# zpelgrims/pota

Measured on AMD Instinct MI355X. Metric: bidir redistribution Msamples/s at 4K, double-gauss 50mm, higher is better.
Workload: dtype f64

## Files before the change

include/lentil_hip.h:

```cpp
#ifndef LENTIL_HIP_H
#define LENTIL_HIP_H

#include <stddef.h>
#include <stdint.h>

#ifdef __cplusplus
extern "C" {
#endif

#define LENTIL_ABI_VERSION 1

#define LENTIL_OK 0
#define LENTIL_ERR_INVALID (-1)
#define LENTIL_ERR_HIP (-2)
#define LENTIL_ERR_UNSUPPORTED (-3)
#define LENTIL_ERR_NOMEM (-4)

#define LENTIL_THINLENS 0
#define LENTIL_POLYNOMIAL_OPTICS 1
#define LENTIL_UNIT_MM 0
#define LENTIL_UNIT_CM 1
#define LENTIL_UNIT_DM 2
#define LENTIL_UNIT_M 3
#define LENTIL_FILTER_GAUSSIAN 0
// ... 208 lines not shown

int lentil_hip_accum_buffer(lentil_hip_ctx *ctx, void **device_ptr, uint64_t *n_floats);
int lentil_hip_stream(lentil_hip_ctx *ctx, void **hip_stream);

int lentil_hip_comm_unique_id(uint8_t id[128]);
int lentil_hip_comm_init(lentil_hip_ctx *ctx, const uint8_t id[128], int rank, int world);
int lentil_hip_comm_destroy(lentil_hip_ctx *ctx);
int lentil_hip_allreduce(lentil_hip_ctx *ctx);
int lentil_hip_exchange_bands(lentil_hip_ctx *ctx, const int32_t *bounds, int32_t visit_rows, int32_t sparse,
                              int32_t *band_lo, int32_t *band_hi);
int lentil_hip_exchange_stats(lentil_hip_ctx *ctx, uint64_t *bytes_sent, uint64_t *bytes_received);
int lentil_hip_exchange_counts(lentil_hip_ctx *ctx, uint64_t *fixed_form, uint64_t *pairs_overflowed);
int lentil_hip_degenerate_stats(lentil_hip_ctx *ctx, uint32_t *degenerate, uint64_t *flagged_pixels, uint64_t *nodes_sent,
                                uint64_t *nodes_received, uint64_t *passes_rerun);
int lentil_hip_streams_concurrent(lentil_hip_ctx *ctx, int *concurrent);
int lentil_hip_box_probe(lentil_hip_ctx *ctx, double probe[6]);

typedef struct lentil_crypto_visits {
  uint64_t n;
  uint32_t n_crypto;
  uint32_t entries;
  const float *hash[LENTIL_MAX_CRYPTO];
  const float *weight[LENTIL_MAX_CRYPTO];
} lentil_crypto_visits;
int lentil_hip_alloc_crypto(lentil_hip_ctx *ctx, uint32_t n_crypto, uint32_t slots_per_pixel);
int lentil_hip_upload_crypto(lentil_hip_ctx *ctx, const lentil_crypto_visits *c);
int lentil_hip_bind_crypto(lentil_hip_ctx *ctx, const lentil_crypto_visits *c);
int lentil_hip_visits_begin_crypto(lentil_hip_ctx *ctx, uint32_t entries);
int lentil_hip_visits_append_crypto(lentil_hip_ctx *ctx, const lentil_visits *part, const lentil_crypto_visits *caches,
                                    uint64_t *ticket);
int lentil_hip_download_crypto(lentil_hip_ctx *ctx, uint32_t crypto, uint32_t rank, float *host_rgba, uint8_t *host_has_rank);
int lentil_hip_download_crypto_table(lentil_hip_ctx *ctx, uint32_t crypto, uint32_t *slots_per_pixel, uint32_t *host_id_bits,
                                     float *host_weight, float *host_total);

int lentil_hip_get_counters(lentil_hip_ctx *ctx, lentil_counters *out);
int lentil_hip_last_timing(lentil_hip_ctx *ctx, float ms[3]);
int lentil_hip_last_launches(lentil_hip_ctx *ctx, uint32_t n[2]);
int lentil_hip_batch_model_stats(lentil_hip_ctx *ctx, uint64_t stats[4]);
int lentil_hip_process_stats(uint64_t stats[4]);
int lentil_hip_process_stall_notes(char *buf, uint64_t capacity);
typedef struct lentil_probe_segment {
  float origin[3];
  float target[3];
} lentil_probe_segment;
typedef void (*lentil_probe_fn)(void *user, uint64_t n, const lentil_probe_segment *segments, uint8_t *occluded);
int lentil_hip_set_occlusion_probe(lentil_hip_ctx *ctx, lentil_probe_fn fn, void *user, const float *camera_to_world);
int lentil_hip_probe_stats(lentil_hip_ctx *ctx, uint64_t stats[3]);

int lentil_hip_set_async(lentil_hip_ctx *ctx, int on);
int lentil_hip_pass_totals(lentil_hip_ctx *ctx, lentil_pass_totals *out, int reset);
int lentil_hip_debug_batch_estimate(lentil_hip_ctx *ctx, uint64_t n, const float *cs_xyz, uint32_t samples, float *out);
int lentil_hip_set_draw_log(lentil_hip_ctx *ctx, uint64_t capacity);
int lentil_hip_download_draw_log(lentil_hip_ctx *ctx, lentil_draw_record *out, uint64_t capacity,
                                 uint64_t *n_records);

#define LENTIL_RAYS_DEVICE_POINTERS 1u
#define LENTIL_RAYS_NO_DIFFERENTIALS 2u
typedef struct lentil_camera_ray_batch {
  uint64_t n;
  uint64_t first_ray;
  const float *in;
  float *out;
  int32_t *tries;
  double lambda;
  float exposure;
  uint32_t rng_seed;
  uint32_t flags;
} lentil_camera_ray_batch;
int lentil_hip_camera_rays(lentil_hip_ctx *ctx, const lentil_camera_ray_batch *batch);
int lentil_hip_camera_rays_path(lentil_hip_ctx *ctx, int *path);

int lentil_hip_test_y0_intersection(lentil_hip_ctx *ctx, uint64_t n, const double *sensor_shift, double lambda,
                                    double *distance, double *sensor, double *out);
int lentil_hip_test_lt_sample_aperture(lentil_hip_ctx *ctx, uint64_t n, const double *scene,
                                       const double *ap, double lambda, double *sensor,
                                       double *out, double *transmittance);
int lentil_hip_test_trace_bw_po(lentil_hip_ctx *ctx, uint64_t n, const double *target,
                                const int32_t *px, const int32_t *py, const int32_t *attempt,
                                double *sensor_xy, int32_t *ok);
int lentil_hip_test_aperture_sample(lentil_hip_ctx *ctx, uint64_t n, const uint32_t *a,
                                    const uint32_t *b, double *xy);
int lentil_hip_test_xor128_jump(const uint32_t in[4], uint64_t k, uint32_t out[4]);
int lentil_hip_debug_scan_bands(const lentil_params *params, float out[8]);
enum {
  LENTIL_SCAN_DMA2 = 1,
  LENTIL_SCAN_DMA = 2,
  LENTIL_SCAN_DMA_MULTI = 3,
  LENTIL_SCAN_UNIFORM = 4,
  LENTIL_SCAN_UNIFORM_MULTI = 5,
  LENTIL_SCAN_RUNS = 6,
  LENTIL_SCAN_RAGGED = 7
};
int lentil_hip_debug_last_scan(lentil_hip_ctx *ctx, uint32_t out[4]);

#ifdef __cplusplus
}
#endif
#endif
```

pota_amd/capi.py:

```python
import ctypes as C
import os

import numpy as np

from . import _abi

_PKG = os.path.dirname(os.path.abspath(__file__))
LIB_PATH = os.environ.get("LENTIL_HIP_LIB") or os.path.join(_PKG, "liblentil_hip.so")

EXPORTS = [
    "lentil_hip_abi_version", "lentil_hip_create", "lentil_hip_destroy", "lentil_hip_last_error", "lentil_hip_last_redo_note",
    "lentil_hip_set_params", "lentil_hip_set_lens", "lentil_hip_set_bokeh", "lentil_hip_alloc_frame", "lentil_hip_set_camera_motion", "lentil_hip_set_camera_shutter",
    "lentil_hip_upload_visits", "lentil_hip_bind_visits", "lentil_hip_clear_frame",
    "lentil_hip_redistribute", "lentil_hip_resolve", "lentil_hip_sync", "lentil_hip_download_aov",
    "lentil_hip_download_accum", "lentil_hip_download_records", "lentil_hip_accum_buffer", "lentil_hip_stream",
    "lentil_hip_set_closest_exchange", "lentil_hip_zkey_buffer", "lentil_hip_closest_gather",
    "lentil_hip_touched_rows", "lentil_hip_merge_rows", "lentil_hip_resolve_rows",
    "lentil_hip_pack_rows", "lentil_hip_merge_packed_rows", "lentil_hip_compact_rows", "lentil_hip_merge_sparse",
    "lentil_hip_get_counters", "lentil_hip_last_timing", "lentil_hip_last_launches", "lentil_hip_set_draw_log",
    "lentil_hip_batch_model_stats", "lentil_hip_process_stats", "lentil_hip_process_stall_notes", "lentil_hip_set_async", "lentil_hip_pass_totals", "lentil_hip_set_occlusion_probe", "lentil_hip_probe_stats", "lentil_hip_debug_batch_estimate", "lentil_hip_box_probe",
    "lentil_hip_lens_jit_status", "lentil_hip_lens_jit_wait", "lentil_hip_debug_lens_jit_source", "lentil_hip_debug_lens_jit_compile",
    "lentil_hip_download_draw_log", "lentil_hip_test_lt_sample_aperture",
    "lentil_hip_test_trace_bw_po", "lentil_hip_test_aperture_sample", "lentil_hip_debug_scan_bands", "lentil_hip_debug_last_scan",
    "lentil_hip_lens_is_compiled", "lentil_hip_set_lens_mode",
    "lentil_hip_focus_search", "lentil_hip_test_y0_intersection", "lentil_hip_camera_rays", "lentil_hip_camera_rays_path",
    "lentil_hip_set_xor128_state", "lentil_hip_get_xor128_state", "lentil_hip_tl_chroma_stats", "lentil_hip_test_xor128_jump",
    "lentil_hip_host_alloc", "lentil_hip_host_free", "lentil_hip_visits_begin", "lentil_hip_visits_append",
    "lentil_hip_visits_wait", "lentil_hip_visits_end",
    "lentil_hip_comm_unique_id", "lentil_hip_comm_init", "lentil_hip_comm_destroy", "lentil_hip_allreduce",
    "lentil_hip_exchange_bands", "lentil_hip_exchange_stats", "lentil_hip_exchange_counts", "lentil_hip_degenerate_stats", "lentil_hip_streams_concurrent",
    "lentil_hip_alloc_crypto", "lentil_hip_upload_crypto", "lentil_hip_bind_crypto", "lentil_hip_download_crypto",
    "lentil_hip_download_crypto_table", "lentil_hip_visits_begin_crypto", "lentil_hip_visits_append_crypto",
]

SCAN_DMA2, SCAN_DMA, SCAN_DMA_MULTI, SCAN_UNIFORM, SCAN_UNIFORM_MULTI, SCAN_RUNS, SCAN_RAGGED = range(1, 8)
SCAN_NAMES = {SCAN_DMA2: "dma2", SCAN_DMA: "dma", SCAN_DMA_MULTI: "dma_multi", SCAN_UNIFORM: "uniform",
              SCAN_UNIFORM_MULTI: "uniform_multi", SCAN_RUNS: "runs", SCAN_RAGGED: "ragged"}

_lib = None


def process_stats():
    lib = load_library()
    n = (C.c_uint64 * 4)()
    rc = lib.lentil_hip_process_stats(n)
    if rc:
        raise RuntimeError("lentil_hip_process_stats: %d" % rc)
    return tuple(int(x) for x in n)


def process_stall_notes():
    lib = load_library()
    buf = C.create_string_buffer(1 << 14)
    lib.lentil_hip_process_stall_notes(buf, 1 << 14)
    return buf.value.decode(errors="replace")


def _tea8(v0, v1):
    v0 = np.asarray(v0, np.uint32).copy()
    v1 = np.broadcast_to(np.asarray(v1, np.uint32), v0.shape).copy()
    s0 = np.uint32(0)
    with np.errstate(over="ignore"):
        for _ in range(8):
            s0 = np.uint32((int(s0) + 0x9E3779B9) & 0xFFFFFFFF)
            v0 += ((v1 << np.uint32(4)) + np.uint32(0xA341316C)) ^ (v1 + s0) ^ ((v1 >> np.uint32(5)) + np.uint32(0xC8013EA4))
            v1 += ((v0 << np.uint32(4)) + np.uint32(0xAD90777D)) ^ (v0 + s0) ^ ((v0 >> np.uint32(5)) + np.uint32(0x7E95761E))
    return v0


def ray_rng_state(ray_id, seed):
    rid = np.asarray(ray_id, np.uint32)
    w = [_tea8(rid, np.uint32(int(seed) & 0xFFFFFFFF))]
    for _ in range(3):
        w.append(_tea8(rid, w[-1]))
    st = np.stack(w, -1)
    st[~st.any(-1)] = np.array([123456789, 362436069, 521288629, 88675123], np.uint32)
    return st


class LentilError(RuntimeError):
    def __init__(self, code, msg):
        super().__init__("lentil_hip error %d: %s" % (code, msg))
        self.code = code


def load_library():
    global _lib
    if _lib is not None:
        return _lib
    if os.environ.get("LENTIL_NO_TORCH") != "1":
        try:
            import torch
        except ImportError:
            pass
    if not os.path.exists(LIB_PATH):
        raise FileNotFoundError(
            "%s is missing: build it with `python -c 'import __graft_entry__ as g; g.build()'`" % LIB_PATH)
    lib = C.CDLL(LIB_PATH)
    vp, u32, u64, i = C.c_void_p, C.c_uint32, C.c_uint64, C.c_int
    sig = {
        "lentil_hip_abi_version": (i, []),
        "lentil_hip_create": (i, [i, C.POINTER(vp)]),
        "lentil_hip_destroy": (i, [vp]),
        "lentil_hip_last_error": (C.c_char_p, [vp]),
        "lentil_hip_last_redo_note": (C.c_char_p, [vp]),
        "lentil_hip_set_params": (i, [vp, C.POINTER(_abi.Params)]),
# ... 584 lines not shown
```

pota_amd/csrc/lentil_hip.hip:

```cpp
#include <hip/hip_runtime.h>
#include <hip/hip_ext.h>

#include <algorithm>
#include <atomic>
#include <chrono>
#include <cmath>
#include <cstdio>
#include <cstdlib>
#include <cstring>
#include <deque>
#include <mutex>
#include <new>
#include <string>
#include <vector>

#include "lentil_kernels.h"
#include "lentil_closest_replay.h"
#include "lentil_tl_chroma_mgpu.h"
#include "lentil_lens_jit.h"
#include "lentil_camera_rays.h"
#include "generated/embedded_sources.inc"

#define LENTIL_API extern "C" __attribute__((visibility("default")))

// ... 1738 lines not shown
  int rc;
  if (ctx->F.dir && (rc = fold_direct(ctx, 0, ctx->F.np, true))) return rc;
  if (ctx->dir_dirty && !(region && *region == ctx->dir_region)) {
    const lentil_hip_ctx::DirRegion &r = ctx->dir_region;
    const uint64_t rows = r.ppr ? (r.npix + r.ppr - 1) / r.ppr : 0;
    uint64_t row_lo = (uint64_t)(r.y0 < 0 ? 0 : r.y0);
    uint64_t row_hi = rows ? row_lo + (rows - 1) * (r.row_stride ? r.row_stride : 1) + 1 : row_lo;
    if (row_hi > ctx->P.yres) row_hi = ctx->P.yres;
    if (row_hi > row_lo)
      HIP_TRY(ctx, hipMemsetAsync(ctx->d_dir + row_lo * ctx->P.xres * ctx->F.stride, 0,
                                  (row_hi - row_lo) * ctx->P.xres * ctx->F.stride * sizeof(float), ctx->stream));
    ctx->dir_dirty = false;
  }
  if (region) {
    if (!ctx->d_dir) {
      const uint64_t nfl = ctx->F.np * ctx->F.stride;
      HIP_TRY(ctx, hipMalloc(&ctx->d_dir, nfl * sizeof(float)));
      HIP_TRY(ctx, hipMemsetAsync(ctx->d_dir, 0, nfl * sizeof(float), ctx->stream));
    }
    ctx->F.dir = ctx->d_dir;
    ctx->dir_dirty = true;
    ctx->dir_region = *region;
    if (ctx->cleared_since_pass) {
      if (!ctx->d_touched) {
        const uint64_t n = touched_bytes(ctx->F.np);
        HIP_TRY(ctx, hipMalloc(&ctx->d_touched, n));
        HIP_TRY(ctx, hipMemsetAsync(ctx->d_touched, 0, n, ctx->stream));
      }
      ctx->F.touched = ctx->d_touched;
      ctx->F.touched_px = ctx->d_touched + touched_px_offset(ctx->F.np);
    }
  } else {
    untrust_touched(ctx);
  }
  ctx->cleared_since_pass = false;
  return LENTIL_OK;
}

static ScanBands scan_bands(const lentil_params &P) {
  ScanBands B;
  for (int i = 0; i < 2; ++i) { B.in_lo[i] = 1.0f; B.in_hi[i] = -1.0f; B.out_lo[i] = 1.0f; B.out_hi[i] = -1.0f; }
  B.out_lo[0] = -INFINITY; B.out_hi[0] = INFINITY;
  float fd = (float)P.focus_distance, A = (float)P.aperture_radius;
  if (P.cameraType == LENTIL_POLYNOMIAL_OPTICS) fd = (float)((double)fd / 10.0);
  else A = (float)((double)A * 10.0);
  const float f = P.focal_length;
  const float ifd = (-f * -fd) / (-f + -fd);
  const double a = std::fabs((double)A), c0 = 1.0 + (double)ifd / (double)f, c1 = (double)ifd;
  if (!(a > 0.0) || !std::isfinite(a) || !std::isfinite(c0) || !std::isfinite(c1) || c1 == 0.0 || !(f > 0.0f)) return B;
  const double eps = 1e-3 + 1e-5 * a;
  if (!(eps < 0.25)) return B;
  auto up = [](double v) { float r = (float)v; if ((double)r < v) r = std::nextafter(r, INFINITY); return r; };
  auto down = [](double v) { float r = (float)v; if ((double)r > v) r = std::nextafter(r, -INFINITY); return r; };
  auto pieces = [&](double t, bool inner, float lo[2], float hi[2]) {
    double ua = (c0 - t / a) / c1, ub = (c0 + t / a) / c1;
    if (ua > ub) std::swap(ua, ub);
    lo[0] = lo[1] = 1.0f; hi[0] = hi[1] = -1.0f;
    const double big = inner ? 1e30 : (double)INFINITY;
    if (ua > 0.0 || ub < 0.0) {
      const double zl = 1.0 / ub, zh = 1.0 / ua;
      lo[0] = inner ? up(std::max(zl, -big)) : down(zl);
      hi[0] = inner ? down(std::min(zh, big)) : up(zh);
    } else {
      if (ua < 0.0) { lo[0] = inner ? (float)-big : -INFINITY; hi[0] = inner ? down(1.0 / ua) : up(1.0 / ua); }
      if (ub > 0.0) { lo[1] = inner ? up(1.0 / ub) : down(1.0 / ub); hi[1] = inner ? (float)big : INFINITY; }
      if (!inner && (ua == 0.0 || ub == 0.0)) { lo[0] = -INFINITY; hi[0] = INFINITY; }
    }
  };
  ScanBands R = B;
  pieces(0.4 * (1.0 - eps), true, R.in_lo, R.in_hi);
  pieces(0.4 * (1.0 + eps), false, R.out_lo, R.out_hi);
  for (int i = 0; i < 2; ++i)
    if (std::isnan(R.in_lo[i]) || std::isnan(R.in_hi[i]) || std::isnan(R.out_lo[i]) || std::isnan(R.out_hi[i])) return B;
  return R;
}

LENTIL_API int lentil_hip_debug_scan_bands(const lentil_params *P, float out[8]) {
  if (!P || !out) return LENTIL_ERR_INVALID;
  const ScanBands B = scan_bands(*P);
  for (int i = 0; i < 2; ++i) { out[i] = B.in_lo[i]; out[2 + i] = B.in_hi[i]; out[4 + i] = B.out_lo[i]; out[6 + i] = B.out_hi[i]; }
  return LENTIL_OK;
}

struct ScanPlan {
  ScanArgs sa{};
  size_t lds = 0;
  uint64_t n_tiles = 0;
  bool multi = false;
  bool dma = false;
  bool dma2 = false;
  bool dma_multi = false;
  uint32_t M = 0;
};

static uint32_t dma_multi_ring(const lentil_hip_ctx *) {
  static const int forced = getenv("LENTIL_DMA_MULTI_RING") ? atoi(getenv("LENTIL_DMA_MULTI_RING")) : 0;
  return forced == 3 ? 3u : 2u;
}
static uint32_t dma_multi_blocks_per_cu(const lentil_hip_ctx *ctx) {
  static const int forced = getenv("LENTIL_DMA_MULTI_BLOCKS") ? atoi(getenv("LENTIL_DMA_MULTI_BLOCKS")) : 0;
  if (forced >= 1 && forced <= 4) return (uint32_t)forced;
  const size_t one = (size_t)4 * dma_multi_wave_f4(ctx->V.n_extra, dma_multi_ring(ctx)) * 16 + 4 * kWaveQueueLds * sizeof(uint2);
  return 2u * one + 2u * 10u * 1024u <= 160u * 1024u ? 2u : 1u;
}
static size_t dma_multi_lds(const lentil_hip_ctx *ctx) {
  return (size_t)4 * dma_multi_wave_f4(ctx->V.n_extra, dma_multi_ring(ctx)) * 16 + 4 * kWaveQueueLds * sizeof(uint2);
}

static bool dma_multi_applies(const lentil_hip_ctx *ctx) {
  static const bool allowed = !(getenv("LENTIL_SCAN_DMA_MULTI") && getenv("LENTIL_SCAN_DMA_MULTI")[0] == '0');
  const uint32_t M = ctx->V.visits_per_pixel;
  return allowed && ctx->scan_dma && M > 0 && M <= 64 && ctx->V.n_extra > 0 && !ctx->V.inv_density && !ctx->F.zkey && !ctx->F.zkey_dbg &&
         ctx->F.closest_mask == 0 && ctx->V.cam.n < 2 && ctx->V.n % M == 0 && dma_multi_lds(ctx) <= 160u * 1024u;
}

static size_t solve_block_lds(lentil_hip_ctx *ctx) {
  const bool straight = ctx->use_generated && (lentil_hip_lens_is_compiled(ctx) || jit_function(ctx, false, true) != nullptr);
  return straight ? 29184u : 53760u;
}

static int plan_scan(lentil_hip_ctx *ctx, ScanPlan &pl) {
  ScanArgs &sa = pl.sa;
  sa.P = ctx->P;
  sa.lens_length = ctx->have_lens ? ctx->hlens.length : 0.0;
  sa.V = ctx->V;
  sa.F = ctx->F;
  const uint32_t M = ctx->V.visits_per_pixel;
  pl.M = M;
  if (M) {
    uint32_t ppt = 64;
    uint64_t lds_budget = (ctx->V.n_extra ? 24ull : 48ull) * 1024ull;
    if (const char *e = getenv("LENTIL_SCAN_LDS_KB")) lds_budget = strtoull(e, nullptr, 10) * 1024ull;
    while (ppt > 1 && (uint64_t)ppt * M * 20ull * 4ull > lds_budget) ppt >>= 1;
    if ((uint64_t)ppt * M * 20ull * 4ull > 150ull * 1024ull)
      return fail(ctx, LENTIL_ERR_UNSUPPORTED, "visits_per_pixel too large for the LDS staging area");
    sa.ppt = ppt;
    sa.tv_pad = ppt * M;
    pl.lds = (size_t)sa.tv_pad * 20 * 4 + 4 * kWaveQueueLds * sizeof(uint2);
    pl.multi = ctx->V.n_extra > 0 && M <= 64 && !getenv("LENTIL_SCAN_SINGLE_COLUMN");
    if (pl.multi) {
      ppt = 64 / M;
      sa.ppt = ppt;
      sa.tv_pad = ppt * M;
      const size_t wave_f4 = (size_t)ctx->F.n_aovs * kMultiPlane + 16 + (size_t)ppt * (ctx->F.stride / 4);
      pl.lds = 4 * wave_f4 * 16 + 4 * kWaveQueueLds * sizeof(uint2);
    }
    uint32_t dma_ring = kDmaRing;
    if (const char *e = getenv("LENTIL_DMA_RING")) { const int r = atoi(e); if (r >= 2 && r <= 8) dma_ring = (uint32_t)r; }
    const size_t dma_lds = (size_t)4 * dma_wave_f4(M, dma_ring) * 16 + 4 * kWaveQueueLds * sizeof(uint2);
    pl.dma = ctx->scan_dma && ctx->V.n_extra == 0 && !ctx->V.inv_density && !ctx->F.zkey && !ctx->F.zkey_dbg && ctx->V.cam.n < 2 &&
             ctx->V.n % M == 0 && dma_lds <= 80u * 1024u;
    if (pl.dma) {
      ppt = 64;
      sa.ring = dma_ring;
      sa.ppt = ppt;
      sa.tv_pad = ppt * M;
      pl.lds = dma_lds;
      pl.multi = false;
      static const bool dma2_allowed = !(getenv("LENTIL_SCAN_DMA2") && getenv("LENTIL_SCAN_DMA2")[0] == '0');
      const size_t dma2_lds = (size_t)4 * dma2_wave_f4(M) * 16 + 4 * kWaveQueueLds * sizeof(uint2);
      const size_t solve_lds = (size_t)ctx->stream_blocks * solve_block_lds(ctx);
      const uint64_t ppr = ctx->V.pixels_per_row;
      pl.dma2 = dma2_allowed && M >= 2 && ppr >= 2 && ppr < (1ull << 31) && ctx->V.n / M < (1ull << 31) &&
                dma2_lds + (ctx->stream_mode ? solve_lds : 0) <= 160u * 1024u;
      if (pl.dma2) {
        pl.lds = dma2_lds;
// ... 2436 lines not shown
```

pota_amd/csrc/lentil_kernels.h:

```cpp
#pragma once
#include "lentil_device.h"
#include "lentil_batch_model.h"
#include "generated/lens_registry.h"

using namespace lentil;

struct DevCounters {
  unsigned long long work_count;
  unsigned long long sum_samples;
  unsigned long long redistributed;
  unsigned long long attempted;
  unsigned long long accepted;
  unsigned long long overflow;
  unsigned long long log_count;
  unsigned long long newton_iters;
  unsigned long long tries;
  unsigned long long lane_rounds;
  unsigned long long slow_solves;
  unsigned long long fallback;
  unsigned long long rounds_used;
  unsigned int n_tasks[2];
  unsigned int task_head[2];
  unsigned int n_active[2];
  unsigned int active_head[2];
// ... 680 lines not shown
  nskip[lane] = 0u;
  auto issue_ring = [&](uint64_t v0, uint32_t g) {
    const uint64_t v = v0 + (uint64_t)g * 64u + lane;
    const uint64_t vl = v < V.n ? v : v_last;
    float4 *slot = ring + (size_t)(g % R) * 192u;
    lds_dma16(V.pos_z + vl, slot);
    lds_dma16(V.volume_ignore + vl, slot + 64);
    lds_dma16(V.transmission + vl, slot + 128);
  };

  while (true) {
    uint32_t t4 = 0;
    if (lane == 0) t4 = atomicAdd(&a.ctr->tile_next, 4u);
    t4 = __builtin_amdgcn_readfirstlane(t4);
    if (a.tile_begin + (uint64_t)t4 >= n_tiles) break;
    const uint64_t tile4 = a.tile_begin + (uint64_t)scan_order(a, t4, 4u);
    const uint64_t tile4_end = tile4 + 4u < n_tiles ? tile4 + 4u : n_tiles;
    for (uint64_t tile = tile4; tile < tile4_end; ++tile) {
      const uint64_t pix0 = tile * 64u;
      const uint64_t v0 = pix0 * M;
      for (uint32_t g = 0; g < M; ++g) {
        const uint64_t v = v0 + (uint64_t)g * 64u + lane;
        lds_dma16(V.rgba + (v < V.n ? v : v_last), srgba + (size_t)g * 64u);
      }
      for (uint32_t g = 0; g < R && g < M; ++g) issue_ring(v0, g);
      for (uint32_t g = 0; g < M; ++g) {
        const uint32_t behind = (M - 1u - g) < (R - 1u) ? (M - 1u - g) : (R - 1u);
        wait_vmcnt(3u * behind);
        float4 pz, vi, tr;
        lds_read_slot(ring + (size_t)(g % R) * 192u + lane, pz, vi, tr);
        const uint32_t e = g * 64u + lane;
        const uint64_t v = v0 + e;
        const bool valid = v < V.n;
        bool flagged = false;
        int samples = 0;
        if (valid) {
          flagged = visit_redistributes(a.P, a.lens_length, pz, vi, tr, a.P.inverse_sample_density,
                                        [&]() { return V.raydir_time[v]; }, V.cam);
          if (flagged)
            samples = visit_prologue(a.P, a.lens_length, srgba[e], pz, V.raydir_time[v], vi, tr, a.P.inverse_sample_density, V.cam).samples;
        }
        if (flagged || !valid) {
          srgba[e] = make_float4(0.f, 0.f, 0.f, 0.f);
          atomicAdd(&nskip[e / M], 1u);
        }
        wq.push(flagged, (uint32_t)v, (uint32_t)samples, a);
        if (g + R < M) {
          __builtin_amdgcn_fence(__ATOMIC_RELEASE, "wavefront", "local");
          issue_ring(v0, g + R);
        }
      }
      __builtin_amdgcn_fence(__ATOMIC_RELEASE, "wavefront", "local");
      __builtin_amdgcn_wave_barrier();
      __builtin_amdgcn_fence(__ATOMIC_ACQUIRE, "wavefront", "local");
      const uint64_t pix = pix0 + lane;
      const uint32_t skipped = nskip[lane];
      nskip[lane] = 0u;
      if (pix < n_pixels) {
        float4 s = make_float4(0.f, 0.f, 0.f, 0.f);
        for (uint32_t j = 0; j < M; ++j) {
          const float4 c = srgba[lane * M + j];
          s.x += (c.x + 0.0f) * w; s.y += (c.y + 0.0f) * w; s.z += (c.z + 0.0f) * w; s.w += (c.w + 0.0f) * w;
        }
        float ws = 0.f;
        const uint32_t cnt = M - skipped;
        for (uint32_t j = 0; j < cnt; ++j) ws += w;
        const int px = V.pixel_x0 + (int)(pix % V.pixels_per_row);
        const int py = V.pixel_y0 + (int)(pix / V.pixels_per_row) * (int)V.pixel_row_stride;
        const uint64_t lin = (uint64_t)px + (uint64_t)py * xres;
        dir4[lin * 2u] = s;
        dir4[lin * 2u + 1u] = make_float4(ws, 0.f, 0.f, 0.f);
      }
      __builtin_amdgcn_fence(__ATOMIC_RELEASE, "wavefront", "local");
      __builtin_amdgcn_wave_barrier();
      wq.end_tile(a);
    }
    if (lane == 0) tl_add(TL_SCAN_TILES, (uint32_t)(tile4_end - tile4));
  }
  wq.finish(a);
  scan_block_done(a);
}

__host__ __device__ constexpr uint32_t dma2_wave_f4(uint32_t M) { return 2u * M * 64u + 2u * 192u + 16u; }
LD_DEV float4 lds_read_f4(const float4 *p);

LD_DEV void dma2_col(const float4 *ubase, uint32_t lane16, float4 *lds_uniform) {
  typedef const __attribute__((address_space(1))) void *gptr_t;
  typedef __attribute__((address_space(3))) void *lptr_t;
  __builtin_amdgcn_global_load_lds((gptr_t)(const void *)(reinterpret_cast<const char *>(ubase) + lane16), (lptr_t)(void *)lds_uniform, 16, 0, 2);
}
LD_DEV void lds_read_3f4(const float4 *p, float4 &c0, float4 &c1, float4 &c2) {
  typedef float v4f __attribute__((ext_vector_type(4)));
  typedef const __attribute__((address_space(3))) void *lptr_t;
  const uint32_t addr = (uint32_t)(size_t)(lptr_t)(const void *)p;
  v4f x, y, z;
  asm volatile("ds_read_b128 %0, %3\n\tds_read_b128 %1, %3 offset:16\n\tds_read_b128 %2, %3 offset:32\n\ts_waitcnt lgkmcnt(0)"
               : "=&v"(x), "=&v"(y), "=&v"(z)
               : "v"(addr)
               : "memory");
  c0 = make_float4(x.x, x.y, x.z, x.w); c1 = make_float4(y.x, y.y, y.z, y.w); c2 = make_float4(z.x, z.y, z.z, z.w);
}

LD_DEV int coc_below_by_bands(const ScanBands &B, float cz) {
  const bool in0 = cz >= B.in_lo[0] && cz <= B.in_hi[0];
  const bool in1 = cz >= B.in_lo[1] && cz <= B.in_hi[1];
  const bool out0 = cz >= B.out_lo[0] && cz <= B.out_hi[0];
  const bool out1 = cz >= B.out_lo[1] && cz <= B.out_hi[1];
  if (in0 || in1) return 1;
  if (out0 || out1) return 2;
  return 0;
}

__global__ __launch_bounds__(256) void scan_dma2_kernel(ScanArgs a) {
  LENTIL_TL_SPAN(SPAN_SCAN);
  extern __shared__ float4 smem[];
  if (blockIdx.x < a.skip_blocks) { scan_block_done(a); return; }
  const uint32_t lane = threadIdx.x & 63u, wave = (uint32_t)__builtin_amdgcn_readfirstlane((int)(threadIdx.x >> 6));
  const VisitsDev &V = a.V;
  const uint32_t M = V.visits_per_pixel;
  const uint32_t wave_f4 = dma2_wave_f4(M);
  float4 *rg = smem + (size_t)wave * wave_f4;
  float4 *ring = rg + (size_t)2u * M * 64u;
  uint32_t *nskip = reinterpret_cast<uint32_t *>(ring + 384u);
  uint2 *qmem = reinterpret_cast<uint2 *>(smem + (size_t)4u * wave_f4);
  WaveQueue wq;
  wq.init(qmem + (size_t)wave * kWaveQueueLds);
  __builtin_amdgcn_s_setprio(3);

  const uint32_t lane16 = lane * 16u;
  const uint32_t TV = 64u * M;
  const uint64_t full_end = (V.n / TV) < a.tile_end ? (V.n / TV) : a.tile_end;
  const float w = 1.0f * a.P.inverse_sample_density;
  float ws_full = 0.f;
  for (uint32_t j = 0; j < M; ++j) ws_full += w;
  float4 *dir4 = reinterpret_cast<float4 *>(a.F.dir);
  const uint32_t xres = a.P.xres;
  const float mz0 = a.P.world_to_camera[0][2], mz1 = a.P.world_to_camera[1][2], mz2 = a.P.world_to_camera[2][2], mz3 = a.P.world_to_camera[3][2];
  float scale = 1.0f;
  if (a.P.unitModel == LENTIL_UNIT_MM) scale = 0.1f;
  else if (a.P.unitModel == LENTIL_UNIT_DM) scale = 10.0f;
  else if (a.P.unitModel == LENTIL_UNIT_M) scale = 100.0f;
  const bool never = a.P.adaptive_sampling && a.P.inverse_sample_density > 0.2f;
  const double inside_lens = a.lens_length * 0.1;
  const bool po = a.P.cameraType == LENTIL_POLYNOMIAL_OPTICS;

  nskip[lane] = 0u;
  auto issue_ring = [&](uint64_t v_group, uint32_t slot) {
    float4 *s = ring + (size_t)slot * 192u;
    dma2_col(V.pos_z + v_group, lane16, s);
    dma2_col(V.volume_ignore + v_group, lane16, s + 64);
    dma2_col(V.transmission + v_group, lane16, s + 128);
  };

  auto do_tile = [&](uint64_t tile, bool has_next, uint64_t next_tile, uint32_t buf, uint32_t par) {
    const uint64_t v0 = tile * TV;
    const uint64_t nv0 = next_tile * TV;
    float4 *srgba = rg + (size_t)buf * M * 64u;
    float4 *nrgba = rg + (size_t)(buf ^ 1u) * M * 64u;
    bool tile_any = false;
    for (uint32_t g = 0; g < M; ++g) {
      if (has_next) asm volatile("s_waitcnt vmcnt(5)" ::: "memory");
      else if (g + 1u < M) asm volatile("s_waitcnt vmcnt(3)" ::: "memory");
      else asm volatile("s_waitcnt vmcnt(0)" ::: "memory");
      const uint32_t slot = (par + g) & 1u;
      float4 pz, vi, tr;
      lds_read_slot(ring + (size_t)slot * 192u + lane, pz, vi, tr);
      if (g + 2u < M) issue_ring(v0 + (uint64_t)(g + 2u) * 64u, slot);
      else if (has_next) issue_ring(nv0 + (uint64_t)(g + 2u - M) * 64u, slot);
      if (has_next) dma2_col(V.rgba + nv0 + (uint64_t)g * 64u, lane16, nrgba + (size_t)g * 64u);
      const float wx = pz.x, wy = pz.y, wz = pz.z, depth = pz.w;
      const bool small = fabsf(wx) < kAiEpsilon && fabsf(wy) < kAiEpsilon && fabsf(wz) < kAiEpsilon;
      const bool far = (depth == kAiInfinite) || small;
      const float cz = (wx * mz0 + wy * mz1 + wz * mz2 + mz3) * scale;
      const int below = coc_below_by_bands(a.bands, cz);
      bool flagged;
      if (__ballot((far && a.P.enable_skydome) || below == 2) == 0ull) {
        bool r = !never && !far;
        if (fmaxf(fmaxf(vi.x, vi.y), vi.z) > 0.0f) r = false;
        if (!a.P.enable_bidir_transmission && fmaxf(fmaxf(tr.x, tr.y), tr.z) > 0.0f) r = false;
        if (vi.w > 0.0f) r = false;
        if (below == 1) r = false;
        if (po && (double)fabsf(cz) < inside_lens) r = false;
        flagged = r;
      } else {
        const uint64_t v = v0 + (uint64_t)g * 64u + lane;
        flagged = visit_redistributes(a.P, a.lens_length, pz, vi, tr, a.P.inverse_sample_density,
                                      [&]() { return V.raydir_time[v]; }, V.cam);
      }
      if (__ballot(flagged)) {
        tile_any = true;
        const uint32_t e = g * 64u + lane;
        const uint64_t v = v0 + e;
        int samples = 0;
        if (flagged) {
          samples = visit_prologue(a.P, a.lens_length, lds_read_f4(srgba + e), pz, V.raydir_time[v], vi, tr, a.P.inverse_sample_density, V.cam).samples;
          srgba[e] = make_float4(0.f, 0.f, 0.f, 0.f);
          atomicAdd(&nskip[e / M], 1u);
        }
        wq.push(flagged, (uint32_t)v, (uint32_t)samples, a);
      }
    }
    typedef float v2f __attribute__((ext_vector_type(2)));
    v2f s01 = {0.f, 0.f}, s23 = {0.f, 0.f};
    const v2f w2 = {w, w};
    const float4 *mine = srgba + (size_t)lane * M;
    uint32_t j = 0;
    for (; j + 3u <= M; j += 3u) {
      float4 c0, c1, c2;
      lds_read_3f4(mine + j, c0, c1, c2);
      v2f p;
      p = (v2f){c0.x, c0.y} * w2; s01 += p; p = (v2f){c0.z, c0.w} * w2; s23 += p;
      p = (v2f){c1.x, c1.y} * w2; s01 += p; p = (v2f){c1.z, c1.w} * w2; s23 += p;
      p = (v2f){c2.x, c2.y} * w2; s01 += p; p = (v2f){c2.z, c2.w} * w2; s23 += p;
    }
    for (; j < M; ++j) {
      const float4 c0 = lds_read_f4(mine + j);
      v2f p;
      p = (v2f){c0.x, c0.y} * w2; s01 += p; p = (v2f){c0.z, c0.w} * w2; s23 += p;
    }
    float ws = ws_full;
    if (tile_any) {
      asm volatile("s_waitcnt vmcnt(0)" ::: "memory");
      __builtin_amdgcn_fence(__ATOMIC_RELEASE, "wavefront", "local");
      __builtin_amdgcn_wave_barrier();
      __builtin_amdgcn_fence(__ATOMIC_ACQUIRE, "wavefront", "local");
      const uint32_t skipped = nskip[lane];
      nskip[lane] = 0u;
      ws = 0.f;
      for (uint32_t q = 0; q < M - skipped; ++q) ws += w;
    }
    {
      const uint32_t pix = (uint32_t)(tile * 64u) + lane;
      const uint32_t row = __umulhi(pix, a.ppr_magic) >> a.ppr_shift;
      const uint32_t col = pix - row * V.pixels_per_row;
      const int px = V.pixel_x0 + (int)col;
      const int py = V.pixel_y0 + (int)row * (int)V.pixel_row_stride;
      const uint64_t lin = (uint64_t)px + (uint64_t)py * xres;
      dir4[lin * 2u] = make_float4(s01.x, s01.y, s23.x, s23.y);
      dir4[lin * 2u + 1u] = make_float4(ws, 0.f, 0.f, 0.f);
    }
    if (tile_any) {
      __builtin_amdgcn_fence(__ATOMIC_RELEASE, "wavefront", "local");
      __builtin_amdgcn_wave_barrier();
      wq.end_tile(a);
    }
  };

  const uint64_t n_full = full_end > a.tile_begin ? full_end - a.tile_begin : 0ull;
  const uint32_t n_runs = (uint32_t)((n_full + 3u) / 4u);
  const uint32_t W = (gridDim.x - a.skip_blocks) * 4u;
  const uint32_t R = n_runs / W;
  const uint32_t n_lvl = (R >= 2u ? 1u : 0u) + (R >= 4u ? 1u : 0u) + (R >= 8u ? 1u : 0u) + (R >= 16u ? 1u : 0u);
  const uint32_t lb1 = (R >> 1) * W, lb2 = lb1 + (R >> 2) * W, lb3 = lb2 + (R >> 3) * W, lb4 = lb3 + (R >> 4) * W;
  auto run_first = [&](uint32_t r) { return a.tile_begin + (uint64_t)(a.outside_in ? ((r & 1u) ? n_runs - 1u - (r >> 1) : (r >> 1)) : r) * 4u; };
  auto run_len = [&](uint64_t first) { return (uint32_t)(full_end - first < 4u ? full_end - first : 4u); };
  uint32_t buf = 0, par = 0;
  while (true) {
    uint32_t t = 0;
    if (lane == 0) t = atomicAdd(&a.ctr->tile_next, 1u);
    t = (uint32_t)__builtin_amdgcn_readfirstlane(t);
    uint32_t r, runs_left, stride;
    if (t < n_lvl * W) {
      const uint32_t l = t / W;
      r = (l == 0u ? 0u : (l == 1u ? lb1 : (l == 2u ? lb2 : lb3))) + (t - l * W);
      runs_left = R >> (l + 1u);
      stride = W;
    } else {
      r = lb4 + (t - n_lvl * W);
      runs_left = 1u;
      stride = 0u;
      if (r >= n_runs) break;
    }
    uint64_t tile = run_first(r);
    uint32_t left = run_len(tile);
    {
      const uint64_t v0 = tile * TV;
      for (uint32_t g = 0; g < M; ++g) dma2_col(V.rgba + v0 + (uint64_t)g * 64u, lane16, rg + (size_t)buf * M * 64u + (size_t)g * 64u);
      issue_ring(v0, par);
      if (M > 1u) issue_ring(v0 + 64u, par ^ 1u);
      asm volatile("s_waitcnt vmcnt(0)" ::: "memory");
    }
    while (true) {
      bool has_next = false;
      uint64_t next_tile = tile;
      uint32_t next_left = 0;
      if (left > 1u) { has_next = true; next_tile = tile + 1u; next_left = left - 1u; }
      else if (runs_left > 1u) {
        has_next = true;
        next_tile = run_first(r + stride);
        next_left = run_len(next_tile);
      }
      do_tile(tile, has_next, next_tile, buf, par);
      if (lane == 0) tl_add(TL_SCAN_TILES, 1u);
      buf ^= 1u;
      par = (par + M) & 1u;
      if (left == 1u) { r += stride; --runs_left; }
      if (!has_next) break;
      tile = next_tile; left = next_left;
    }
  }
  if (a.tile_end > full_end && blockIdx.x == a.skip_blocks && wave == 0) {
    const uint64_t tile = full_end;
    const uint64_t n_pixels = V.n / M;
    const uint64_t pix = tile * 64u + lane;
    asm volatile("s_waitcnt vmcnt(0)" ::: "memory");
    float4 s = make_float4(0.f, 0.f, 0.f, 0.f);
    float ws = 0.f;
    for (uint32_t j = 0; j < M; ++j) {
      const uint64_t v = pix * M + j;
      const bool valid = pix < n_pixels;
      bool flagged = false;
      int samples = 0;
      float4 c = make_float4(0.f, 0.f, 0.f, 0.f);
      if (valid) {
        const float4 pz = V.pos_z[v], vi = V.volume_ignore[v], tr = V.transmission[v];
        c = V.rgba[v];
        flagged = visit_redistributes(a.P, a.lens_length, pz, vi, tr, a.P.inverse_sample_density, [&]() { return V.raydir_time[v]; }, V.cam);
        if (flagged) samples = visit_prologue(a.P, a.lens_length, c, pz, V.raydir_time[v], vi, tr, a.P.inverse_sample_density, V.cam).samples;
      }
      if (valid && !flagged) { s.x += c.x * w; s.y += c.y * w; s.z += c.z * w; s.w += c.w * w; ws += w; }
      wq.push(flagged, (uint32_t)v, (uint32_t)samples, a);
    }
    if (pix < n_pixels) {
      const int px = V.pixel_x0 + (int)(pix % V.pixels_per_row);
      const int py = V.pixel_y0 + (int)(pix / V.pixels_per_row) * (int)V.pixel_row_stride;
      const uint64_t lin = (uint64_t)px + (uint64_t)py * xres;
      dir4[lin * 2u] = s;
      dir4[lin * 2u + 1u] = make_float4(ws, 0.f, 0.f, 0.f);
    }
    wq.end_tile(a);
  }
  asm volatile("s_waitcnt vmcnt(0)" ::: "memory");
  wq.finish(a);
  scan_block_done(a);
}

LD_DEV float4 lds_read_f4(const float4 *p) {
  typedef float v4f __attribute__((ext_vector_type(4)));
  typedef const __attribute__((address_space(3))) void *lptr_t;
  const uint32_t addr = (uint32_t)(size_t)(lptr_t)(const void *)p;
  v4f x;
  asm volatile("ds_read_b128 %0, %1\n\ts_waitcnt lgkmcnt(0)" : "=&v"(x) : "v"(addr) : "memory");
  return make_float4(x.x, x.y, x.z, x.w);
}
LD_DEV void lds_read_4f4(const float4 *p, float4 c[4]) {
  typedef float v4f __attribute__((ext_vector_type(4)));
  typedef const __attribute__((address_space(3))) void *lptr_t;
  const uint32_t addr = (uint32_t)(size_t)(lptr_t)(const void *)p;
  v4f x, y, z, w;
  asm volatile("ds_read_b128 %0, %4\n\tds_read_b128 %1, %4 offset:16\n\tds_read_b128 %2, %4 offset:32\n\tds_read_b128 %3, %4 offset:48\n\t"
               "s_waitcnt lgkmcnt(0)"
               : "=&v"(x), "=&v"(y), "=&v"(z), "=&v"(w)
               : "v"(addr)
               : "memory");
  c[0] = make_float4(x.x, x.y, x.z, x.w); c[1] = make_float4(y.x, y.y, y.z, y.w);
  c[2] = make_float4(z.x, z.y, z.z, z.w); c[3] = make_float4(w.x, w.y, w.z, w.w);
}
LD_DEV float4 global_read_f4_untracked(const float4 *p) {
  typedef float v4f __attribute__((ext_vector_type(4)));
  v4f x;
  asm volatile("global_load_dwordx4 %0, %1, off\n\ts_waitcnt vmcnt(0)" : "=&v"(x) : "v"(p) : "memory");
  return make_float4(x.x, x.y, x.z, x.w);
}
constexpr uint32_t kDmaMultiRun = 16;
constexpr uint32_t kDmaMultiCol = 65;
__host__ __device__ constexpr uint32_t dma_multi_wave_f4(uint32_t n_extra, uint32_t ring) { return ring * (4u + n_extra) * kDmaMultiCol; }

__global__ __launch_bounds__(256) void scan_dma_multi_kernel(ScanArgs a) {
  LENTIL_TL_SPAN(SPAN_SCAN);
  extern __shared__ float4 smem[];
  const uint32_t lane = threadIdx.x & 63u, wave = threadIdx.x >> 6;
  const VisitsDev &V = a.V;
  const uint32_t M = V.visits_per_pixel, K = V.n_extra, n_aovs = a.F.n_aovs;
  const uint32_t n_cols = 4u + K;
  const uint32_t ppt = a.ppt, TV = ppt * M;
  constexpr uint32_t CS = kDmaMultiCol;
  const uint32_t R = a.ring & 0xFFu;
  float4 *ring = smem + (size_t)wave * dma_multi_wave_f4(K, R);
  uint2 *qmem = reinterpret_cast<uint2 *>(smem + (size_t)4u * dma_multi_wave_f4(K, R));
  WaveQueue wq;
  wq.init(qmem + (size_t)wave * kWaveQueueLds);
  __builtin_amdgcn_s_setprio(3);
  const uint64_t n_pixels = V.n / M;
  const uint64_t n_tiles = a.tile_end;
  const uint32_t xres = a.P.xres, q = a.F.stride >> 2;
  const float w_in = 1.0f * a.P.inverse_sample_density;
  float4 *dir4 = reinterpret_cast<float4 *>(a.F.dir);
  float4 *dummy = a.dummy + lane;
  const uint64_t v_last = V.n - 1;
  const uint32_t n_sum = ppt * q, passes = (n_sum + 63u) / 64u, store_ops = passes;

  auto issue = [&](uint64_t tile, uint32_t si) {
    const uint64_t v = tile * (uint64_t)TV + lane;
    const uint64_t vl = (lane < TV && v < V.n) ? v : v_last;
    float4 *slot = ring + (size_t)si * n_cols * CS;
    if (a.ring & 0x100u) {
      lds_dma16_cached(V.pos_z + vl, slot);
      lds_dma16_cached(V.volume_ignore + vl, slot + CS);
      lds_dma16_cached(V.transmission + vl, slot + 2u * CS);
      lds_dma16_cached(V.rgba + vl, slot + 3u * CS);
      for (uint32_t k = 0; k < K; ++k) lds_dma16_cached(V.extra[k] + vl, slot + (4u + k) * CS);
      return;
    }
    lds_dma16(V.pos_z + vl, slot);
    lds_dma16(V.volume_ignore + vl, slot + CS);
    lds_dma16(V.transmission + vl, slot + 2u * CS);
    lds_dma16(V.rgba + vl, slot + 3u * CS);
    for (uint32_t k = 0; k < K; ++k) lds_dma16(V.extra[k] + vl, slot + (4u + k) * CS);
  };

#ifdef LENTIL_TIMELINE
  uint64_t tacc[6] = {0, 0, 0, 0, 0, 0};
#endif
  while (true) {
    uint32_t t0 = 0;
    if (lane == 0) t0 = atomicAdd(&a.ctr->tile_next, kDmaMultiRun);
    t0 = __builtin_amdgcn_readfirstlane(t0);
    if (a.tile_begin + (uint64_t)t0 >= n_tiles) break;
    const uint64_t run0 = a.tile_begin + (uint64_t)scan_order(a, t0, kDmaMultiRun);
    const uint64_t run1 = run0 + kDmaMultiRun < n_tiles ? run0 + kDmaMultiRun : n_tiles;
    for (uint32_t g = 0; g < R && run0 + g < run1; ++g) issue(run0 + g, g);
    uint32_t si = 0;
    for (uint64_t tile = run0; tile < run1; ++tile) {
      const uint32_t behind = (uint32_t)(run1 - 1u - tile) < R - 1u ? (uint32_t)(run1 - 1u - tile) : R - 1u;
      const uint32_t before = (uint32_t)(tile - run0) < R - 1u ? (uint32_t)(tile - run0) : R - 1u;
#ifdef LENTIL_TIMELINE
      const uint64_t tp0 = clock64();
#endif
      wait_vmcnt(behind * n_cols + before * store_ops);
#ifdef LENTIL_TIMELINE
      const uint64_t tp1 = clock64();
#endif
      const float4 *slot = ring + (size_t)si * n_cols * CS;
      const uint64_t pix0 = tile * ppt;
      const uint64_t v = tile * (uint64_t)TV + lane;
      const bool valid = lane < TV && v < V.n;
      float4 pz, vi, tr;
      lds_read_slot<CS * 16u>(slot + lane, pz, vi, tr);
      bool flagged = false;
      int samples = 0;
      if (valid) {
        flagged = visit_redistributes(a.P, a.lens_length, pz, vi, tr, a.P.inverse_sample_density,
                                      [&]() { return global_read_f4_untracked(V.raydir_time + v); });
        if (flagged)
          samples = visit_prologue(a.P, a.lens_length, lds_read_f4(slot + 3u * CS + lane), pz,
// ... 3006 lines not shown
```

Before: 37350.

## Add adaptive lean scan mode streaming only positions with on-demand attribute fetch

The dma2 scan kernel gains a lean mode that prefetches only pos_z through a deeper LDS ring of up to six slots. It loads volume_ignore and transmission directly from global memory only for wave groups that could redistribute. A per-tile hysteresis switches between lean and full prefetch from how many groups were open, and re-primes the ring on each switch, so quiet tiles move less memory traffic. The redistribution checks now pass a static camera-motion descriptor instead of V.cam, which changes behaviour if camera motion is in use. Each mode switch also adds a full memory wait.

```diff
diff --git a/include/lentil_hip.h b/include/lentil_hip.h
--- a/include/lentil_hip.h
+++ b/include/lentil_hip.h
@@ -314,6 +314,7 @@
                                     const uint32_t *b, double *xy);
 int lentil_hip_test_xor128_jump(const uint32_t in[4], uint64_t k, uint32_t out[4]);
 int lentil_hip_debug_scan_bands(const lentil_params *params, float out[8]);
+int lentil_hip_debug_scan_lean_counts(uint32_t out[3]);
 enum {
   LENTIL_SCAN_DMA2 = 1,
   LENTIL_SCAN_DMA = 2,
diff --git a/pota_amd/capi.py b/pota_amd/capi.py
--- a/pota_amd/capi.py
+++ b/pota_amd/capi.py
@@ -21,7 +21,7 @@
     "lentil_hip_batch_model_stats", "lentil_hip_process_stats", "lentil_hip_process_stall_notes", "lentil_hip_set_async", "lentil_hip_pass_totals", "lentil_hip_set_occlusion_probe", "lentil_hip_probe_stats", "lentil_hip_debug_batch_estimate", "lentil_hip_box_probe",
     "lentil_hip_lens_jit_status", "lentil_hip_lens_jit_wait", "lentil_hip_debug_lens_jit_source", "lentil_hip_debug_lens_jit_compile",
     "lentil_hip_download_draw_log", "lentil_hip_test_lt_sample_aperture",
-    "lentil_hip_test_trace_bw_po", "lentil_hip_test_aperture_sample", "lentil_hip_debug_scan_bands", "lentil_hip_debug_last_scan",
+    "lentil_hip_test_trace_bw_po", "lentil_hip_test_aperture_sample", "lentil_hip_debug_scan_bands", "lentil_hip_debug_scan_lean_counts", "lentil_hip_debug_last_scan",
     "lentil_hip_lens_is_compiled", "lentil_hip_set_lens_mode",
     "lentil_hip_focus_search", "lentil_hip_test_y0_intersection", "lentil_hip_camera_rays", "lentil_hip_camera_rays_path",
     "lentil_hip_set_xor128_state", "lentil_hip_get_xor128_state", "lentil_hip_tl_chroma_stats", "lentil_hip_test_xor128_jump",
diff --git a/pota_amd/csrc/lentil_hip.hip b/pota_amd/csrc/lentil_hip.hip
--- a/pota_amd/csrc/lentil_hip.hip
+++ b/pota_amd/csrc/lentil_hip.hip
@@ -1844,6 +1844,12 @@
   return LENTIL_OK;
 }
 
+LENTIL_API int lentil_hip_debug_scan_lean_counts(uint32_t out[3]) {
+  if (!out) return LENTIL_ERR_INVALID;
+  out[0] = kLeanRing; out[1] = kBusyGroups; out[2] = kQuietTiles;
+  return LENTIL_OK;
+}
+
 struct ScanPlan {
   ScanArgs sa{};
   size_t lds = 0;
diff --git a/pota_amd/csrc/lentil_kernels.h b/pota_amd/csrc/lentil_kernels.h
--- a/pota_amd/csrc/lentil_kernels.h
+++ b/pota_amd/csrc/lentil_kernels.h
@@ -786,7 +786,21 @@
 }
 
 __host__ __device__ constexpr uint32_t dma2_wave_f4(uint32_t M) { return 2u * M * 64u + 2u * 192u + 16u; }
+constexpr uint32_t kLeanRing = 6;
+constexpr uint32_t kBusyGroups = 2;
+constexpr uint32_t kQuietTiles = 2;
 LD_DEV float4 lds_read_f4(const float4 *p);
+LD_DEV void global_read_2f4_untracked(const float4 *p, const float4 *q, uint32_t lane16, float4 &x, float4 &y);
+
+LD_DEV void wait_vmcnt_lean(uint32_t n) {
+#define LENTIL_VMCNT_CASE(N) case N: asm volatile("s_waitcnt vmcnt(" #N ")" ::: "memory"); break;
+  switch (n) {
+    LENTIL_VMCNT_CASE(1) LENTIL_VMCNT_CASE(2) LENTIL_VMCNT_CASE(3) LENTIL_VMCNT_CASE(4) LENTIL_VMCNT_CASE(5) LENTIL_VMCNT_CASE(6)
+    LENTIL_VMCNT_CASE(7) LENTIL_VMCNT_CASE(8) LENTIL_VMCNT_CASE(9) LENTIL_VMCNT_CASE(10) LENTIL_VMCNT_CASE(11) LENTIL_VMCNT_CASE(12)
+    default: asm volatile("s_waitcnt vmcnt(0)" ::: "memory"); break;
+  }
+#undef LENTIL_VMCNT_CASE
+}
 
 LD_DEV void dma2_col(const float4 *ubase, uint32_t lane16, float4 *lds_uniform) {
   typedef const __attribute__((address_space(1))) void *gptr_t;
@@ -847,6 +861,7 @@
   const bool never = a.P.adaptive_sampling && a.P.inverse_sample_density > 0.2f;
   const double inside_lens = a.lens_length * 0.1;
   const bool po = a.P.cameraType == LENTIL_POLYNOMIAL_OPTICS;
+  const CamMotion still{nullptr, 0u, 0.0f, 1.0f};
 
   nskip[lane] = 0u;
   auto issue_ring = [&](uint64_t v_group, uint32_t slot) {
@@ -856,40 +871,62 @@
     dma2_col(V.transmission + v_group, lane16, s + 128);
   };
 
-  auto do_tile = [&](uint64_t tile, bool has_next, uint64_t next_tile, uint32_t buf, uint32_t par) {
+  const uint32_t D = M < kLeanRing ? M : kLeanRing;
+  uint32_t ls = 0;
+  auto do_tile = [&](bool lean, uint64_t tile, bool has_next, uint64_t next_tile, uint32_t buf, uint32_t par) -> uint32_t {
     const uint64_t v0 = tile * TV;
     const uint64_t nv0 = next_tile * TV;
     float4 *srgba = rg + (size_t)buf * M * 64u;
     float4 *nrgba = rg + (size_t)(buf ^ 1u) * M * 64u;
     bool tile_any = false;
+    uint32_t open_groups = 0;
     for (uint32_t g = 0; g < M; ++g) {
-      if (has_next) asm volatile("s_waitcnt vmcnt(5)" ::: "memory");
-      else if (g + 1u < M) asm volatile("s_waitcnt vmcnt(3)" ::: "memory");
-      else asm volatile("s_waitcnt vmcnt(0)" ::: "memory");
-      const uint32_t slot = (par + g) & 1u;
       float4 pz, vi, tr;
-      lds_read_slot(ring + (size_t)slot * 192u + lane, pz, vi, tr);
-      if (g + 2u < M) issue_ring(v0 + (uint64_t)(g + 2u) * 64u, slot);
-      else if (has_next) issue_ring(nv0 + (uint64_t)(g + 2u - M) * 64u, slot);
+      if (lean) {
+        if (has_next) wait_vmcnt_lean(2u * D - 1u);
+        else wait_vmcnt_lean(M - 1u - g < D - 1u ? M - 1u - g : D - 1u);
+        float4 *s = ring + (size_t)ls * 64u;
+        pz = lds_read_f4(s + lane);
+        if (g + D < M) dma2_col(V.pos_z + v0 + (uint64_t)(g + D) * 64u, lane16, s);
+        else if (has_next) dma2_col(V.pos_z + nv0 + (uint64_t)(g + D - M) * 64u, lane16, s);
+        ls = ls + 1u == D ? 0u : ls + 1u;
+        vi = tr = make_float4(0.f, 0.f, 0.f, 0.f);
+      } else {
+        if (has_next) asm volatile("s_waitcnt vmcnt(5)" ::: "memory");
+        else if (g + 1u < M) asm volatile("s_waitcnt vmcnt(3)" ::: "memory");
+        else asm volatile("s_waitcnt vmcnt(0)" ::: "memory");
+        const uint32_t slot = (par + g) & 1u;
+        lds_read_slot(ring + (size_t)slot * 192u + lane, pz, vi, tr);
+        if (g + 2u < M) issue_ring(v0 + (uint64_t)(g + 2u) * 64u, slot);
+        else if (has_next) issue_ring(nv0 + (uint64_t)(g + 2u - M) * 64u, slot);
+      }
       if (has_next) dma2_col(V.rgba + nv0 + (uint64_t)g * 64u, lane16, nrgba + (size_t)g * 64u);
       const float wx = pz.x, wy = pz.y, wz = pz.z, depth = pz.w;
       const bool small = fabsf(wx) < kAiEpsilon && fabsf(wy) < kAiEpsilon && fabsf(wz) < kAiEpsilon;
       const bool far = (depth == kAiInfinite) || small;
       const float cz = (wx * mz0 + wy * mz1 + wz * mz2 + mz3) * scale;
       const int below = coc_below_by_bands(a.bands, cz);
-      bool flagged;
-      if (__ballot((far && a.P.enable_skydome) || below == 2) == 0ull) {
-        bool r = !never && !far;
-        if (fmaxf(fmaxf(vi.x, vi.y), vi.z) > 0.0f) r = false;
-        if (!a.P.enable_bidir_transmission && fmaxf(fmaxf(tr.x, tr.y), tr.z) > 0.0f) r = false;
-        if (vi.w > 0.0f) r = false;
-        if (below == 1) r = false;
-        if (po && (double)fabsf(cz) < inside_lens) r = false;
-        flagged = r;
-      } else {
-        const uint64_t v = v0 + (uint64_t)g * 64u + lane;
-        flagged = visit_redistributes(a.P, a.lens_length, pz, vi, tr, a.P.inverse_sample_density,
-                                      [&]() { return V.raydir_time[v]; }, V.cam);
+      const bool ask = __ballot((far && a.P.enable_skydome) || below == 2) != 0ull;
+      bool open = !far && below != 1;
+      if (lean) open = open && !never && !(po && (double)fabsf(cz) < inside_lens);
+      const bool group_open = ask || __ballot(open) != 0ull;
+      if (group_open) ++open_groups;
+      bool flagged = false;
+      if (!lean || group_open) {
+        const uint64_t vg = v0 + (uint64_t)g * 64u, v = vg + lane;
+        if (lean) global_read_2f4_untracked(V.volume_ignore + vg, V.transmission + vg, lane16, vi, tr);
+        if (!ask) {
+          bool r = !never && !far;
+          if (fmaxf(fmaxf(vi.x, vi.y), vi.z) > 0.0f) r = false;
+          if (!a.P.enable_bidir_transmission && fmaxf(fmaxf(tr.x, tr.y), tr.z) > 0.0f) r = false;
+          if (vi.w > 0.0f) r = false;
+          if (below == 1) r = false;
+          if (po && (double)fabsf(cz) < inside_lens) r = false;
+          flagged = r;
+        } else {
+          flagged = visit_redistributes(a.P, a.lens_length, pz, vi, tr, a.P.inverse_sample_density,
+                                        [&]() { return V.raydir_time[v]; }, still);
+        }
       }
       if (__ballot(flagged)) {
         tile_any = true;
@@ -897,13 +934,14 @@
         const uint64_t v = v0 + e;
         int samples = 0;
         if (flagged) {
-          samples = visit_prologue(a.P, a.lens_length, lds_read_f4(srgba + e), pz, V.raydir_time[v], vi, tr, a.P.inverse_sample_density, V.cam).samples;
+          samples = visit_prologue(a.P, a.lens_length, lds_read_f4(srgba + e), pz, V.raydir_time[v], vi, tr, a.P.inverse_sample_density, still).samples;
           srgba[e] = make_float4(0.f, 0.f, 0.f, 0.f);
           atomicAdd(&nskip[e / M], 1u);
         }
         wq.push(flagged, (uint32_t)v, (uint32_t)samples, a);
       }
     }
+    if (lean && D == M) wait_vmcnt_lean(has_next ? 2u * M : 0u);
     typedef float v2f __attribute__((ext_vector_type(2)));
     v2f s01 = {0.f, 0.f}, s23 = {0.f, 0.f};
     const v2f w2 = {w, w};
@@ -948,6 +986,16 @@
       __builtin_amdgcn_wave_barrier();
       wq.end_tile(a);
     }
+    return open_groups;
+  };
+  auto prime_ring = [&](bool for_lean, uint64_t v0, uint32_t par) {
+    if (for_lean) {
+      for (uint32_t g = 0; g < D; ++g) dma2_col(V.pos_z + v0 + (uint64_t)g * 64u, lane16, ring + (size_t)g * 64u);
+      ls = 0;
+    } else {
+      issue_ring(v0, par);
+      if (M > 1u) issue_ring(v0 + 64u, par ^ 1u);
+    }
   };
 
   const uint64_t n_full = full_end > a.tile_begin ? full_end - a.tile_begin : 0ull;
@@ -959,6 +1007,8 @@
   auto run_first = [&](uint32_t r) { return a.tile_begin + (uint64_t)(a.outside_in ? ((r & 1u) ? n_runs - 1u - (r >> 1) : (r >> 1)) : r) * 4u; };
   auto run_len = [&](uint64_t first) { return (uint32_t)(full_end - first < 4u ? full_end - first : 4u); };
   uint32_t buf = 0, par = 0;
+  bool lean = true;
+  uint32_t quiet = 0;
   while (true) {
     uint32_t t = 0;
     if (lane == 0) t = atomicAdd(&a.ctr->tile_next, 1u);
@@ -980,8 +1030,7 @@
     {
       const uint64_t v0 = tile * TV;
       for (uint32_t g = 0; g < M; ++g) dma2_col(V.rgba + v0 + (uint64_t)g * 64u, lane16, rg + (size_t)buf * M * 64u + (size_t)g * 64u);
-      issue_ring(v0, par);
-      if (M > 1u) issue_ring(v0 + 64u, par ^ 1u);
+      prime_ring(lean, v0, par);
       asm volatile("s_waitcnt vmcnt(0)" ::: "memory");
     }
     while (true) {
@@ -994,10 +1043,22 @@
         next_tile = run_first(r + stride);
         next_left = run_len(next_tile);
       }
-      do_tile(tile, has_next, next_tile, buf, par);
+      const uint32_t open_groups = do_tile(lean, tile, has_next, next_tile, buf, par);
       if (lane == 0) tl_add(TL_SCAN_TILES, 1u);
       buf ^= 1u;
       par = (par + M) & 1u;
+      const bool busy = open_groups >= kBusyGroups;
+      quiet = busy ? 0u : quiet + 1u;
+      const bool next_lean = lean ? !busy : quiet >= kQuietTiles;
+      if (next_lean != lean) {
+        lean = next_lean;
+        quiet = 0u;
+        if (has_next) {
+          asm volatile("s_waitcnt vmcnt(0)" ::: "memory");
+          prime_ring(lean, next_tile * TV, par);
+          asm volatile("s_waitcnt vmcnt(0)" ::: "memory");
+        }
+      }
       if (left == 1u) { r += stride; --runs_left; }
       if (!has_next) break;
       tile = next_tile; left = next_left;
@@ -1065,6 +1126,13 @@
   v4f x;
   asm volatile("global_load_dwordx4 %0, %1, off\n\ts_waitcnt vmcnt(0)" : "=&v"(x) : "v"(p) : "memory");
   return make_float4(x.x, x.y, x.z, x.w);
+}
+LD_DEV void global_read_2f4_untracked(const float4 *p, const float4 *q, uint32_t lane16, float4 &x, float4 &y) {
+  typedef float v4f __attribute__((ext_vector_type(4)));
+  v4f u, v;
+  asm volatile("global_load_dwordx4 %0, %4, %2\n\tglobal_load_dwordx4 %1, %4, %3\n\ts_waitcnt vmcnt(0)"
+               : "=&v"(u), "=&v"(v) : "s"(p), "s"(q), "v"(lane16) : "memory");
+  x = make_float4(u.x, u.y, u.z, u.w); y = make_float4(v.x, v.y, v.z, v.w);
 }
 constexpr uint32_t kDmaMultiRun = 16;
 constexpr uint32_t kDmaMultiCol = 65;
```

Result: faster. 42150 (median of 6 runs) (+12.8%).
